# OSUrobotics/KinovaGrasping

Hardware: AMD Instinct MI355X
Metric: env-steps/sec (whole node) at 4096 envs/GPU (higher is better)
Workload: dtype f32

## Files before the change

kinovagrasping_amd/build.py:

```python
from __future__ import annotations

import os
import shutil
import subprocess
from pathlib import Path

PKG = Path(__file__).resolve().parent
CSRC = PKG / "csrc"
LIB = PKG / "libkinova_sim.so"
LIB_MG = PKG / "libkinova_sim_mg.so"
SOURCES = ["ks_api.hip", "ks_rollout.hip", "ks_mlp.hip", "ks_xchg.hip"]
HEADERS = ["ks_math.h", "ks_model.h", "ks_model_host.h", "ks_core.h", "ks_obs.h", "ks_env.h", "../../include/kinova_sim.h", "../../include/kinova_rollout.h"]


def hipcc_path() -> str:
    for cand in (os.environ.get("HIPCC"), shutil.which("hipcc"), "/opt/rocm/bin/hipcc"):
        if cand and Path(cand).exists():
            return cand
    raise RuntimeError("hipcc not found (need ROCm; this package has no CPU build)")


def needs_build(lib: Path = LIB) -> bool:
    if not lib.exists():
        return True
    t = lib.stat().st_mtime
    return any((CSRC / f).stat().st_mtime > t for f in SOURCES + HEADERS)


def build(force: bool = False, verbose: bool = False, multi_geom: bool | None = None) -> Path:
    for mg in ([False, True] if multi_geom is None else [bool(multi_geom)]):
        lib = LIB_MG if mg else LIB
        if not force and not needs_build(lib):
            continue
        cmd = [hipcc_path(), "--offload-arch=gfx950", "-O3", "-std=c++17", "-fPIC", "-shared"] + (["-DKS_MULTI_GEOM"] if mg else []) + \
              ["-o", str(lib)] + [str(CSRC / s) for s in SOURCES]
        if verbose:
            cmd.insert(1, "-Rpass-analysis=kernel-resource-usage")
        subprocess.check_call(cmd, cwd=str(CSRC))
    return LIB_MG if multi_geom else LIB
```

kinovagrasping_amd/csrc/ks_api.hip:

```cpp
#include <hip/hip_runtime.h>

#include <algorithm>
#include <cstdio>
#include <cstdlib>
#include <cstring>
#include <type_traits>
#include <map>
#include <string>
#include <vector>

#include "../../include/kinova_sim.h"
#include "ks_env.h"
#include "ks_mlp_tile.h"
#include "ks_select.h"
#include "ks_model_host.h"

using namespace ks;

namespace {

constexpr int WAVE = 64;
thread_local std::string g_create_error;

template <typename T> struct StartPool {
// ... 590 lines not shown
                wg_rays<false>(m, *bdev, N, blockIdx.x * epw, epw, (KS_LDS unsigned*)(lds + ((hull_words >> 2) << 2)) KS_RAY_PROF_ARG(nullptr));
                __threadfence_block();
                __syncthreads();
            }
            if (obs_in_step) wg_obs<false>(m, *bdev, N, blockIdx.x * epw, epw, (KS_LDS unsigned*)(lds + ((hull_words >> 2) << 2)), *out);
            if (ray_pool) {
                KS_LDS int* last = (KS_LDS int*)(lds + ((hull_words >> 2) << 2));
                __syncthreads();
                if (threadIdx.x == 0) *last = atomicAdd(&b.rayq[2], 1) == n_wg - 1;
                __syncthreads();
                if (*last) {
                    for (int i = threadIdx.x; i < 2 * n_wg; i += WG) b.rayq[4 + i] = 0;
                    if (threadIdx.x < 4) b.rayq[threadIdx.x] = 0;
                }
            }
        }
    }
}


template <typename T, bool USE_LDS>
__global__ __launch_bounds__(WG) void k_env_step(const Model<T>* __restrict__ models, Buffers<T> b, const Buffers<T>* __restrict__ bdev,
                                                   const T* __restrict__ action, int N, int frame_skip, int iters, int epw, int tap, int rays_in_step,
                                                   int pair_memory, int obs_in_step, const ObsOut<T>* __restrict__ out, int ray_pool, int n_wg) {
    env_step_body<T, USE_LDS>(models, b, bdev, action, N, frame_skip, iters, epw, tap, rays_in_step, pair_memory, obs_in_step, out, ray_pool, n_wg);
}
__global__ __launch_bounds__(WG) KS_STEP_REGS void k_env_step_f32(const Model<float>* __restrict__ models, Buffers<float> b, const Buffers<float>* __restrict__ bdev,
                                                                       const float* __restrict__ action, int N, int frame_skip, int iters, int epw, int tap, int rays_in_step,
                                                                       int pair_memory, int obs_in_step, const ObsOut<float>* __restrict__ out, int ray_pool, int n_wg) {
    env_step_body<float, true>(models, b, bdev, action, N, frame_skip, iters, epw, tap, rays_in_step, pair_memory, obs_in_step, out, ray_pool, n_wg);
}


template <int NT1, int NT2, bool EXACT = false>
__device__ __noinline__ void rollout_policy(const ks_rollout_args* __restrict__ rap, int N, int row_env, KS_LDS float* blocks) {
    const ks_rollout_args& ra = *rap;
    const int S = krsel::S, A = krsel::A;
    kmlp::f32x4(*H1)[kmlp::ROWS] = (kmlp::f32x4(*)[kmlp::ROWS])(float*)blocks;
    kmlp::f32x4(*H2)[kmlp::ROWS] = H1 + NT1 * 4;
    kmlp::f32x4(*Pp)[kmlp::ROWS] = H2 + NT2 * 4;
    const int wave = threadIdx.x >> 6, lane = threadIdx.x & 63;
    long long* vbox = (long long*)(Pp + kmlp::NW);
    for (;;) {
        if (threadIdx.x == 0) vbox[0] = (long long)__hip_atomic_load(ra.actor_ver, __ATOMIC_RELAXED, __HIP_MEMORY_SCOPE_AGENT);
        __syncthreads();
        const long long ver = vbox[0];
        __builtin_amdgcn_fence(__ATOMIC_ACQUIRE, "agent");
        const float* pw = ra.actor_pub + (ver % 3) * ra.actor_stride;
        kmlp::f32x4 z4 = {0.f, 0.f, 0.f, 0.f};
        const bool mine = kmlp::mlp3_rows16<NT1, NT2, true>(wave, lane, (long)row_env, S, 0, ra.h1, ra.h2, A, ra.obs, S, nullptr, 0, pw + ra.off_w1,
                                                            pw + ra.off_b1, pw + ra.off_w2, pw + ra.off_b2, pw + ra.off_w3, nullptr, nullptr, H1, H2, Pp,
                                                            z4);
        float y[4] = {0.f, 0.f, 0.f, 0.f};
        if (mine) {
            const float z[4] = {z4.x, z4.y, z4.z, z4.w};
            const float* b3 = pw + ra.off_b3;
#pragma unroll
            for (int i = 0; i < 4; i++) y[i] = ra.max_action / (1.f + __expf(-(z[i] + b3[i])));
        }
        __syncthreads();
        __builtin_amdgcn_fence(__ATOMIC_ACQUIRE, "agent");
        if (threadIdx.x == 0) vbox[1] = (long long)__hip_atomic_load(ra.actor_ver, __ATOMIC_RELAXED, __HIP_MEMORY_SCOPE_AGENT) - ver;
        __syncthreads();
        const bool stale = vbox[1] >= 2;
        if (stale && threadIdx.x == 0 && ra.repeats) atomicAdd((unsigned long long*)ra.repeats, 1ull);
        if (!stale) {
            if (mine) {
                float nz[4];
                krsel::normal4(ra.seed, (unsigned long long)ra.steps_total[row_env], (uint32_t)row_env, nz);
                krsel::select_one(row_env, N, y, nz, ra.obs, ra.prev_obs, ra.has_prev, ra.t, ra.ready, ra.sigma, ra.max_action, ra.skip_steps, ra.action,
                                  ra.action_t, ra.lifting);
            }
            return;
        }
        __syncthreads();
    }
}

__device__ __noinline__ void rollout_controller(const RolloutController* __restrict__ ctl, const ks_rollout_args* __restrict__ rap, int N, int row_env) {
    if (row_env < 0) return;
    const ks_rollout_args& ra = *rap;
    krsel::controller_one(row_env, N, ctl->mode, ctl->lift_rule, ra.obs, ra.prev_obs, ra.has_prev, ra.t, ra.ready, ctl->init, ra.skip_steps, ra.action,
                          ra.action_t, ra.lifting);
}
__global__ void k_controller_set(RolloutController* rec, RolloutController v, int N) {
// ... 132 lines not shown
            for (int j = 0; j < WARM_WORDS; j++) gw[q].w[j] = pair_memory ? pm[q * WARM_WORDS + j] : 0u;
        }
        lane_env_step(m, hu, *(LaneState<T>*)stp, hq, act, scr, team, snap, frame_skip, iters, ncon, status, (float*)nullptr, stp + NQ + 2 * NV, gw,
                      []() {});
        if (pair_memory) {
            KS_UNROLL
            for (int q = 0; q < WPL; q++) {
                KS_UNROLL
                for (int j = 0; j < WARM_WORDS; j++) pm[q * WARM_WORDS + j] = gw[q].w[j];
            }
        }
        team.sync();
        store_state_team<T, SUBS>(b, env, N, stp, team.sub);
        if (status) atomicOr(&b.status[env], status);
        if (team.sub == 0) b.ncon[env] = ncon;
    }
    __threadfence_block();
    __syncthreads();
    KS_RS(1)
    wg_rays<false>(m, b, N, grp * epw, epw, w KS_RAY_PROF_ARG((long long*)&rap->counters[8 + 4 * 512]));
    __threadfence_block();
    __syncthreads();
    KS_RS(2)
    wg_obs<false>(m, b, N, grp * epw, epw, w, *out);
    __threadfence_block();
    __syncthreads();
    if (active) rollout_store<float>(rap, N, env, team.sub);
    __threadfence_block();
    __syncthreads();
    KS_RS(3)
#undef KS_RS
}

__device__ __forceinline__ long long uniform64(long long v) {
    const unsigned lo = (unsigned)__builtin_amdgcn_readfirstlane((int)(unsigned)v), hi = (unsigned)__builtin_amdgcn_readfirstlane((int)(unsigned)((unsigned long long)v >> 32));
    return (long long)(((unsigned long long)hi << 32) | lo);
}
template <int NT1, int NT2>
__device__ __noinline__ void rollout_policy_wave(const ks_rollout_args* __restrict__ rap, int N, int row_env, KS_LDS float* wblocks) {
    const ks_rollout_args& ra = *rap;
    const int S = krsel::S, A = krsel::A;
    constexpr int NR = 4;
    kmlp::f32x4(*H1)[NR] = (kmlp::f32x4(*)[NR])(float*)wblocks;
    kmlp::f32x4(*H2)[NR] = H1 + NT1 * 4;
    const int lane = threadIdx.x & 63;
    for (;;) {
        const long long ver = uniform64(__hip_atomic_load(ra.actor_ver, __ATOMIC_RELAXED, __HIP_MEMORY_SCOPE_AGENT));
        __builtin_amdgcn_fence(__ATOMIC_ACQUIRE, "agent");
        const float* pw = ra.actor_pub + (ver % 3) * ra.actor_stride;
        kmlp::f32x4 z4 = {0.f, 0.f, 0.f, 0.f};
        const bool mine = kmlp::mlp3_rows_wave<NT1, NT2, true, NR>(lane, (long)row_env, S, ra.h1, ra.h2, A, ra.obs, S, pw + ra.off_w1, pw + ra.off_b1,
                                                                     pw + ra.off_w2, pw + ra.off_b2, pw + ra.off_w3, H1, H2, z4);
        float y[4] = {0.f, 0.f, 0.f, 0.f};
        if (mine) {
            const float z[4] = {z4.x, z4.y, z4.z, z4.w};
            const float* b3 = pw + ra.off_b3;
#pragma unroll
            for (int i = 0; i < 4; i++) y[i] = ra.max_action / (1.f + __expf(-(z[i] + b3[i])));
        }
        __builtin_amdgcn_fence(__ATOMIC_ACQUIRE, "agent");
        const long long ver2 = uniform64(__hip_atomic_load(ra.actor_ver, __ATOMIC_RELAXED, __HIP_MEMORY_SCOPE_AGENT));
        if (ver2 - ver < 2) {
            if (mine) {
                float nz[4];
                krsel::normal4(ra.seed, (unsigned long long)ra.steps_total[row_env], (uint32_t)row_env, nz);
                krsel::select_one(row_env, N, y, nz, ra.obs, ra.prev_obs, ra.has_prev, ra.t, ra.ready, ra.sigma, ra.max_action, ra.skip_steps, ra.action,
                                  ra.action_t, ra.lifting);
            }
            return;
        }
        if (lane == 0 && ra.repeats) atomicAdd((unsigned long long*)ra.repeats, 1ull);
    }
}

template <int NT1, int NT2>
__device__ __forceinline__ void rollout_iter_wave(const Model<float>& m, const Hulls<float>& hu, const Buffers<float>* __restrict__ bdev, int N, int frame_skip,
                                               int iters, int epw, int pair_memory, const ObsOut<float>* __restrict__ out,
                                               const ks_rollout_args* __restrict__ rap, KS_LDS float* blocks, int grp) {
    using T = float;
    using C = Crew<true>;
    const Buffers<T>& b = *bdev;
    const int wave = threadIdx.x >> 6, lane = threadIdx.x & 63;
    const int e = threadIdx.x / LANE_STRIDE;
    const Team<SUBS> team{(int)threadIdx.x % LANE_STRIDE};
    const int env = e < epw ? b.slot_env[grp * epw + e] : -1;
// ... 1106 lines not shown
            out_sent = out;
            ObsOut<T>* slot = pinned_record(capturing, h_out, (unsigned)h_out_next++, captured_out);
            if (!slot) { error = "ks_step: more captured calls than the context keeps output records for"; return KS_ERR_STATE; }
            *slot = out;
            HIPCHK(hipMemcpyAsync(d_out, slot, sizeof out, hipMemcpyHostToDevice, s));
        }
        if (timed) HIPCHK(hipEventRecord(ev0[ev_used], s));
        if constexpr (sizeof(T) == 4)
            hipLaunchKernelGGL(k_env_step_f32, dim3(n_wg), dim3(WG), step_lds, s, d_model, b, (const Buffers<T>*)d_b, (const T*)action, N,
                               cfg.frame_skip, cfg.solver_iterations, lpw, cfg.contact_tap, (int)rays_in_step, (int)(USE_LDS && cfg.pair_memory),
                               (int)obs_in_step, (const ObsOut<T>*)d_out, ray_pool, n_wg);
        else
            hipLaunchKernelGGL((k_env_step<T, USE_LDS>), dim3(n_wg), dim3(WG), step_lds, s, d_model, b, (const Buffers<T>*)d_b, (const T*)action, N,
                               cfg.frame_skip, cfg.solver_iterations, lpw, cfg.contact_tap, (int)rays_in_step, (int)(USE_LDS && cfg.pair_memory),
                               (int)obs_in_step, (const ObsOut<T>*)d_out, ray_pool, n_wg);
        if (timed) { HIPCHK(hipEventRecord(ev1[ev_used], s)); ev_used++; }
        if (!rays_in_step) hipLaunchKernelGGL((k_rays<T>), dim3((N + RAY_ENVS - 1) / RAY_ENVS, NRAY), dim3(WAVE), 0, s, d_model, b, N, 0);
        if (!obs_in_step) hipLaunchKernelGGL((k_obs<T>), dim3(blocks()), dim3(WAVE), 0, s, d_model, b, N, 0, out);
        HIPCHK(hipGetLastError());
        return KS_OK;
    }
    int check_rollout_buffers(int n_iter, const ks_rollout_args* ra) {
        if (!ra || n_iter <= 0 || (ctl_mode == 0 && (!ra->actor_pub || !ra->actor_ver)) || !ra->obs || !ra->prev_obs || !ra->has_prev || !ra->ready || !ra->lifting ||
            !ra->t || !ra->steps_total || !ra->action || !ra->action_t || !ra->reward_out || !ra->done_out || !ra->sim_obs || !ra->sim_reward ||
            !ra->sim_done || !ra->sim_info || !ra->sim_final_obs || !ra->counters) { error = "ks_rollout: NULL argument"; return KS_ERR_INVALID; }
        if (ra->with_replay && (!ra->cur_state || !ra->cur_next || !ra->cur_action || !ra->cur_reward || !ra->cur_not_done || !ra->cur_len ||
                                !ra->cur_sel || !ra->pub_len || ra->horizon <= ra->n_steps)) { error = "ks_rollout: replay buffers"; return KS_ERR_INVALID; }
        return KS_OK;
    }
    int check_rollout_actor(const ks_rollout_args* ra) {
        if (ctl_mode != 0) return KS_OK;
        if ((ra->off_w2 | ra->off_w3 | ra->actor_stride) & 3) { error = "ks_rollout: weight offsets must be multiples of 4 floats"; return KS_ERR_INVALID; }
        if ((ra->h1 | ra->h2) & 3) { error = "ks_rollout: hidden widths must be multiples of 4"; return KS_ERR_INVALID; }
        return KS_OK;
    }
    int send_rollout_records(const ks_rollout_args* ra, hipStream_t s) {
        const ObsOut<T> out{(T*)ra->sim_obs, (T*)ra->sim_reward, ra->sim_done, (T*)ra->sim_info, (T*)ra->sim_final_obs, cfg.horizon, cfg.auto_reset, cfg.obs_env_major};
        const bool capturing = stream_is_capturing(s);
        ObsOut<T>* slot = pinned_record(capturing, h_out, (unsigned)h_out_next++, captured_out);
        if (!slot) { error = "ks_rollout: more captured calls than the context keeps output records for"; return KS_ERR_STATE; }
        *slot = out;
        out_valid = false;
        HIPCHK(hipMemcpyAsync(d_out, slot, sizeof out, hipMemcpyHostToDevice, s));
        ks_rollout_args* rslot = pinned_record(capturing, h_ra, h_ra_next++, captured_ra);
        if (!rslot) { error = "ks_rollout: more captured calls than the context keeps argument records for"; return KS_ERR_STATE; }
        *rslot = *ra;
        HIPCHK(hipMemcpyAsync(d_ra, rslot, sizeof *ra, hipMemcpyHostToDevice, s));
        return KS_OK;
    }
    int rollout_exact(int n_iter, const ks_rollout_args* ra, hipStream_t s) {
#ifdef KS_MULTI_GEOM
        (void)n_iter; (void)ra; (void)s;
        error = "ks_rollout: libkinova_sim_mg.so runs fp32 contexts only (the exact mode, precision 64, is in libkinova_sim.so)";
        return KS_ERR_INVALID;
#else
        int r;
        if ((r = check_rollout_buffers(n_iter, ra))) return r;
        if (!cfg.obs_env_major || !cfg.auto_reset) { error = "ks_rollout needs env-major observations and auto_reset"; return KS_ERR_STATE; }
        if ((r = check_rollout_actor(ra))) return r;
        if (ra->budget_ticks != 0) { error = "ks_rollout: a time budget needs the wave form of the rollout kernel (ks_rollout_plan: KS_PLAN_WAVES); fp64 contexts have none"; return KS_ERR_STATE; }
        const size_t ws_offset = (step_lds + 15) / 16 * 16;
        const size_t policy_bytes = (size_t)(((ra->h1 + 15) / 16 + (ra->h2 + 15) / 16) * 4 + 4) * 16 * 16 + 16;
        const size_t lds = ws_offset + std::max(policy_bytes, (size_t)F64_RAY_BYTES);
        if (lds > 160 * 1024) { error = "ks_rollout: no LDS for the policy beside this object's hull tables"; return KS_ERR_STATE; }
        if ((r = send_rollout_records(ra, s))) return r;
        const int N = cfg.n_envs;
// ... 441 lines not shown
```

kinovagrasping_amd/csrc/ks_mlp.hip:

```cpp
#include <hip/hip_runtime.h>
#include <stdint.h>

#include <type_traits>

#include "../../include/kinova_rollout.h"
#include "../../include/kinova_sim.h"
#include "ks_mlp_tile.h"
#include "ks_select.h"

namespace {

using namespace kmlp;

#ifndef KS_SPLIT_WAVES_PER_EU
#define KS_SPLIT_WAVES_PER_EU 3
#endif

struct SelectArgs {
    const float* obs; const float* prev_obs; const uint8_t* has_prev; const int64_t* t; uint8_t* ready;
    const float* noise; unsigned long long seed; int64_t* rng_state;
    float sigma, max_action; int skip_steps;
    float* action; float* action_t; uint8_t* lifting;
};

template <int NT1, int NT2, bool VEC, bool SEL>
__global__ __launch_bounds__(64 * NW) void k_mlp3(int n, int in_a, int in_b, int h1, int h2, int out_dim, const float* __restrict__ xa, int lda,
                                              const float* __restrict__ xb, int ldb, const float* __restrict__ W1, const float* __restrict__ b1,
                                              const float* __restrict__ W2, const float* __restrict__ b2, const float* __restrict__ W3,
                                              const float* __restrict__ b3, int act, float scale, float* __restrict__ out, float* __restrict__ h1_out,
                                              float* __restrict__ h2_out, SelectArgs sel) {
    __shared__ f32x4 H1[NT1 * 4][ROWS];
    __shared__ f32x4 H2[NT2 * 4][ROWS];
    __shared__ f32x4 P[NW][ROWS];
    const int wave = threadIdx.x >> 6, lane = threadIdx.x & 63, nn = lane & 15;
    const int row = blockIdx.x * ROWS + nn;
    const bool row_ok = row < n;
    unsigned long long rng_step = 0;
    if (SEL && sel.rng_state) rng_step = (unsigned long long)sel.rng_state[0];
    f32x4 z4 = {0.f, 0.f, 0.f, 0.f};
    if (mlp3_rows16<NT1, NT2, VEC>(wave, lane, row_ok ? (long)row : -1L, in_a, in_b, h1, h2, out_dim, xa, lda, xb, ldb, W1, b1, W2, b2, W3, h1_out, h2_out,
                                   H1, H2, P, z4)) {
        const float z[4] = {z4.x, z4.y, z4.z, z4.w};
        float y[4] = {0.f, 0.f, 0.f, 0.f};
        for (int i = 0; i < out_dim; i++) {
            y[i] = z[i] + b3[i];
            if (act == KR_ACT_SIGMOID) y[i] = scale / (1.f + __expf(-y[i]));
            if (out) out[(long)row * out_dim + i] = y[i];
        }
        if (SEL) {
            float nz[4];
            if (sel.noise) {
#pragma unroll
                for (int k = 0; k < 4; k++) nz[k] = sel.noise[(long)row * 4 + k];
            } else {
                krsel::normal4(sel.seed, rng_step, (uint32_t)row, nz);
            }
            krsel::select_one(row, n, y, nz, sel.obs, sel.prev_obs, sel.has_prev, sel.t, sel.ready, sel.sigma, sel.max_action, sel.skip_steps,
                              sel.action, sel.action_t, sel.lifting);
        }
    }
    if (SEL && sel.rng_state) {
        __syncthreads();
        if (threadIdx.x == 0) {
            __threadfence();
            const unsigned ticket = atomicAdd((unsigned*)(sel.rng_state + 1), 1u);
            if (ticket == gridDim.x - 1) {
                sel.rng_state[1] = 0;
                sel.rng_state[0] = (int64_t)(rng_step + 1);
            }
        }
    }
}

template <int NT1, int NT2, bool VEC>
// ... 903 lines not shown
```

kinovagrasping_amd/csrc/ks_mlp_tile.h:

```cpp
#pragma once
#include <hip/hip_runtime.h>
#include <stdint.h>

namespace kmlp {

typedef float f32x4 __attribute__((ext_vector_type(4)));

constexpr int ROWS = 16;
constexpr int KS_IN_MAX = 6;
#ifndef KS_MLP_WAVES
#define KS_MLP_WAVES 4
#endif
constexpr int NW = KS_MLP_WAVES;

template <bool VEC> __device__ __forceinline__ f32x4 load_w4(const float* __restrict__ W, int row, int nrow, int k, int K) {
    f32x4 v = {0.f, 0.f, 0.f, 0.f};
    if (row >= nrow) return v;
    const float* p = W + (long)row * K + k;
    if (VEC && k + 3 < K) return *(const f32x4*)p;
    if (k < K) v.x = p[0];
    if (k + 1 < K) v.y = p[1];
    if (k + 2 < K) v.z = p[2];
    if (k + 3 < K) v.w = p[3];
    return v;
}

__device__ __forceinline__ f32x4 mfma4(f32x4 a, f32x4 b, f32x4 c) {
    c = __builtin_amdgcn_mfma_f32_16x16x4f32(a.x, b.x, c, 0, 0, 0);
    c = __builtin_amdgcn_mfma_f32_16x16x4f32(a.y, b.y, c, 0, 0, 0);
    c = __builtin_amdgcn_mfma_f32_16x16x4f32(a.z, b.z, c, 0, 0, 0);
    c = __builtin_amdgcn_mfma_f32_16x16x4f32(a.w, b.w, c, 0, 0, 0);
    return c;
}

__device__ __forceinline__ f32x4 bias_relu(f32x4 acc, const float* __restrict__ bias, int f, int nfeat) {
    f32x4 r;
    r.x = f < nfeat ? fmaxf(acc.x + bias[f], 0.f) : 0.f;
    r.y = f + 1 < nfeat ? fmaxf(acc.y + bias[f + 1], 0.f) : 0.f;
    r.z = f + 2 < nfeat ? fmaxf(acc.z + bias[f + 2], 0.f) : 0.f;
    r.w = f + 3 < nfeat ? fmaxf(acc.w + bias[f + 3], 0.f) : 0.f;
    return r;
}

template <int NT1, int NT2, bool VEC>
__device__ __forceinline__ bool mlp3_rows16(const int wave, const int lane, const long row, int in_a, int in_b, int h1, int h2, int out_dim,
                                            const float* __restrict__ xa, int lda, const float* __restrict__ xb, int ldb,
                                            const float* __restrict__ W1, const float* __restrict__ b1, const float* __restrict__ W2,
                                            const float* __restrict__ b2, const float* __restrict__ W3, float* __restrict__ h1_out,
                                            float* __restrict__ h2_out, f32x4 (*H1)[ROWS], f32x4 (*H2)[ROWS], f32x4 (*P)[ROWS], f32x4& z4) {
    const int nn = lane & 15, q = lane >> 4;
    const bool row_ok = row >= 0;
    const int in_dim = in_a + in_b;
    f32x4 bx[KS_IN_MAX];
#pragma unroll
    for (int s = 0; s < KS_IN_MAX; s++) {
        float v[4];
#pragma unroll
        for (int j = 0; j < 4; j++) {
            const int k = 16 * s + 4 * q + j;
            float x = 0.f;
            if (row_ok && k < in_a) x = xa[(long)row * lda + k];
            else if (row_ok && k < in_dim) x = xb[(long)row * ldb + (k - in_a)];
            v[j] = x;
        }
        bx[s] = f32x4{v[0], v[1], v[2], v[3]};
    }
    f32x4 w2[NT1];
#pragma unroll
    for (int s = 0; s < NT1; s++) w2[s] = load_w4<VEC>(W2, wave * 16 + nn, wave < NT2 ? h2 : 0, 16 * s + 4 * q, h1);
    {
        f32x4 w1[KS_IN_MAX];
#pragma unroll
        for (int s = 0; s < KS_IN_MAX; s++) w1[s] = load_w4<false>(W1, wave * 16 + nn, wave < NT1 ? h1 : 0, 16 * s + 4 * q, in_dim);
        for (int t = wave; t < NT1; t += NW) {
            f32x4 wn[KS_IN_MAX];
#pragma unroll
            for (int s = 0; s < KS_IN_MAX; s++) wn[s] = load_w4<false>(W1, (t + NW) * 16 + nn, t + NW < NT1 ? h1 : 0, 16 * s + 4 * q, in_dim);
            f32x4 acc0 = {0.f, 0.f, 0.f, 0.f}, acc1 = {0.f, 0.f, 0.f, 0.f};
#pragma unroll
            for (int s = 0; s < KS_IN_MAX; s++) {
                if (s & 1) acc1 = mfma4(w1[s], bx[s], acc1);
                else acc0 = mfma4(w1[s], bx[s], acc0);
            }
            const f32x4 hq = bias_relu(acc0 + acc1, b1, t * 16 + 4 * q, h1);
            H1[t * 4 + q][nn] = hq;
            if (h1_out && row_ok && t * 16 + 4 * q < h1) *(f32x4*)(h1_out + (long)row * h1 + t * 16 + 4 * q) = hq;
#pragma unroll
            for (int s = 0; s < KS_IN_MAX; s++) w1[s] = wn[s];
        }
    }
    __syncthreads();

    f32x4 w3[(NT2 + NW - 1) / NW];
#pragma unroll
    for (int j = 0; j < (NT2 + NW - 1) / NW; j++) w3[j] = load_w4<VEC>(W3, nn, out_dim, 16 * (wave + NW * j) + 4 * q, h2);
    for (int t = wave; t < NT2; t += NW) {
        f32x4 wn[NT1];
#pragma unroll
        for (int s = 0; s < NT1; s++) wn[s] = load_w4<VEC>(W2, (t + NW) * 16 + nn, t + NW < NT2 ? h2 : 0, 16 * s + 4 * q, h1);
        f32x4 acc0 = {0.f, 0.f, 0.f, 0.f}, acc1 = {0.f, 0.f, 0.f, 0.f};
#pragma unroll
        for (int s = 0; s < NT1; s++) {
            if (s & 1) acc1 = mfma4(w2[s], H1[s * 4 + q][nn], acc1);
            else acc0 = mfma4(w2[s], H1[s * 4 + q][nn], acc0);
        }
        const f32x4 hq = bias_relu(acc0 + acc1, b2, t * 16 + 4 * q, h2);
        H2[t * 4 + q][nn] = hq;
        if (h2_out && row_ok && t * 16 + 4 * q < h2) *(f32x4*)(h2_out + (long)row * h2 + t * 16 + 4 * q) = hq;
#pragma unroll
        for (int s = 0; s < NT1; s++) w2[s] = wn[s];
    }
    __syncthreads();

    {
        f32x4 acc = {0.f, 0.f, 0.f, 0.f};
#pragma unroll
        for (int j = 0; j < (NT2 + NW - 1) / NW; j++)
            if (wave + NW * j < NT2) acc = mfma4(w3[j], H2[(wave + NW * j) * 4 + q][nn], acc);
        if (q == 0) P[wave][nn] = acc;
    }
    __syncthreads();
    if (wave == 0 && q == 0 && row_ok) {
        z4 = P[0][nn];
#pragma unroll
        for (int w = 1; w < NW; w++) z4 += P[w][nn];
        return true;
    }
    return false;
}

template <int NT1, int NT2, bool VEC, int NR>
__device__ __forceinline__ bool mlp3_rows_wave(const int lane, const long row, int in_dim, int h1, int h2, int out_dim, const float* __restrict__ xa, int lda,
                                               const float* __restrict__ W1, const float* __restrict__ b1, const float* __restrict__ W2,
                                               const float* __restrict__ b2, const float* __restrict__ W3, f32x4 (*H1)[NR], f32x4 (*H2)[NR], f32x4& z4) {
    const int nn = lane & 15, q = lane >> 4;
    const bool row_ok = row >= 0, col_ok = nn < NR;
    const f32x4 zero = {0.f, 0.f, 0.f, 0.f};
    f32x4 bx[KS_IN_MAX];
#pragma unroll
    for (int s = 0; s < KS_IN_MAX; s++) {
        float v[4];
#pragma unroll
        for (int j = 0; j < 4; j++) {
            const int k = 16 * s + 4 * q + j;
            v[j] = (row_ok && k < in_dim) ? xa[(long)row * lda + k] : 0.f;
        }
        bx[s] = f32x4{v[0], v[1], v[2], v[3]};
    }
    f32x4 w2[NT1];
#pragma unroll
    for (int s = 0; s < NT1; s++) w2[s] = load_w4<VEC>(W2, nn, h2, 16 * s + 4 * q, h1);
    {
        f32x4 w1[KS_IN_MAX];
#pragma unroll
        for (int s = 0; s < KS_IN_MAX; s++) w1[s] = load_w4<false>(W1, nn, h1, 16 * s + 4 * q, in_dim);
        for (int t = 0; t < NT1; t++) {
            f32x4 wn[KS_IN_MAX];
#pragma unroll
            for (int s = 0; s < KS_IN_MAX; s++) wn[s] = load_w4<false>(W1, (t + 1) * 16 + nn, t + 1 < NT1 ? h1 : 0, 16 * s + 4 * q, in_dim);
            f32x4 acc0 = zero, acc1 = zero;
#pragma unroll
            for (int s = 0; s < KS_IN_MAX; s++) {
                if (s & 1) acc1 = mfma4(w1[s], bx[s], acc1);
                else acc0 = mfma4(w1[s], bx[s], acc0);
            }
            const f32x4 hq = bias_relu(acc0 + acc1, b1, t * 16 + 4 * q, h1);
            if (col_ok) H1[t * 4 + q][nn] = hq;
#pragma unroll
            for (int s = 0; s < KS_IN_MAX; s++) w1[s] = wn[s];
        }
    }
    __builtin_amdgcn_fence(__ATOMIC_RELEASE, "wavefront");
    __builtin_amdgcn_wave_barrier();
    __builtin_amdgcn_fence(__ATOMIC_ACQUIRE, "wavefront");

    f32x4 hb[NT1];
#pragma unroll
    for (int s = 0; s < NT1; s++) hb[s] = col_ok ? H1[s * 4 + q][nn] : zero;
    for (int t = 0; t < NT2; t++) {
        f32x4 wn[NT1];
#pragma unroll
        for (int s = 0; s < NT1; s++) wn[s] = load_w4<VEC>(W2, (t + 1) * 16 + nn, t + 1 < NT2 ? h2 : 0, 16 * s + 4 * q, h1);
        f32x4 acc0 = zero, acc1 = zero;
#pragma unroll
        for (int s = 0; s < NT1; s++) {
            if (s & 1) acc1 = mfma4(w2[s], hb[s], acc1);
            else acc0 = mfma4(w2[s], hb[s], acc0);
        }
        const f32x4 hq = bias_relu(acc0 + acc1, b2, t * 16 + 4 * q, h2);
        if (col_ok) H2[t * 4 + q][nn] = hq;
#pragma unroll
        for (int s = 0; s < NT1; s++) w2[s] = wn[s];
    }
    __builtin_amdgcn_fence(__ATOMIC_RELEASE, "wavefront");
    __builtin_amdgcn_wave_barrier();
    __builtin_amdgcn_fence(__ATOMIC_ACQUIRE, "wavefront");

    f32x4 part[NW];
#pragma unroll
    for (int w = 0; w < NW; w++) {
        f32x4 acc = zero;
#pragma unroll
        for (int j = 0; j < (NT2 + NW - 1) / NW; j++)
            if (w + NW * j < NT2) acc = mfma4(load_w4<VEC>(W3, nn, out_dim, 16 * (w + NW * j) + 4 * q, h2), col_ok ? H2[(w + NW * j) * 4 + q][nn] : zero, acc);
        part[w] = acc;
    }
    if (q == 0 && row_ok && col_ok) {
        z4 = part[0];
#pragma unroll
        for (int w = 1; w < NW; w++) z4 += part[w];
        return true;
    }
    return false;
}

}
```

Baseline: 2.731 million.

## Use buffer-resource loads with OOR offsets and double-buffered weight tiles in MLP

Replaces the branchy per-element global weight and input loads in the actor MLP tiles with AMD buffer-resource loads. Out-of-range lanes get an out-of-range offset so the hardware returns zero without branching. Weight and bias tiles are double-buffered (issue next tile, compute current), W3 is preloaded, and scalar parameters are forced uniform via readfirstlane. This adds a host check that observation rows fit in 32-bit byte offsets, and costs more VGPRs for the two tiles held in registers.

```diff
diff --git a/kinovagrasping_amd/build.py b/kinovagrasping_amd/build.py
--- a/kinovagrasping_amd/build.py
+++ b/kinovagrasping_amd/build.py
@@ -10,7 +10,7 @@
 LIB = PKG / "libkinova_sim.so"
 LIB_MG = PKG / "libkinova_sim_mg.so"
 SOURCES = ["ks_api.hip", "ks_rollout.hip", "ks_mlp.hip", "ks_xchg.hip"]
-HEADERS = ["ks_math.h", "ks_model.h", "ks_model_host.h", "ks_core.h", "ks_obs.h", "ks_env.h", "../../include/kinova_sim.h", "../../include/kinova_rollout.h"]
+HEADERS = ["ks_math.h", "ks_model.h", "ks_model_host.h", "ks_core.h", "ks_obs.h", "ks_env.h", "ks_mlp_tile.h", "../../include/kinova_sim.h", "../../include/kinova_rollout.h"]
 
 
 def hipcc_path() -> str:
diff --git a/kinovagrasping_amd/csrc/ks_api.hip b/kinovagrasping_amd/csrc/ks_api.hip
--- a/kinovagrasping_amd/csrc/ks_api.hip
+++ b/kinovagrasping_amd/csrc/ks_api.hip
@@ -646,6 +646,10 @@
 }
 
 
+__device__ __forceinline__ long long uniform64(long long v) {
+    const unsigned lo = (unsigned)__builtin_amdgcn_readfirstlane((int)(unsigned)v), hi = (unsigned)__builtin_amdgcn_readfirstlane((int)(unsigned)((unsigned long long)v >> 32));
+    return (long long)(((unsigned long long)hi << 32) | lo);
+}
 template <int NT1, int NT2, bool EXACT = false>
 __device__ __noinline__ void rollout_policy(const ks_rollout_args* __restrict__ rap, int N, int row_env, KS_LDS float* blocks) {
     const ks_rollout_args& ra = *rap;
@@ -658,13 +662,13 @@
     for (;;) {
         if (threadIdx.x == 0) vbox[0] = (long long)__hip_atomic_load(ra.actor_ver, __ATOMIC_RELAXED, __HIP_MEMORY_SCOPE_AGENT);
         __syncthreads();
-        const long long ver = vbox[0];
+        const long long ver = uniform64(vbox[0]);
         __builtin_amdgcn_fence(__ATOMIC_ACQUIRE, "agent");
         const float* pw = ra.actor_pub + (ver % 3) * ra.actor_stride;
         kmlp::f32x4 z4 = {0.f, 0.f, 0.f, 0.f};
-        const bool mine = kmlp::mlp3_rows16<NT1, NT2, true>(wave, lane, (long)row_env, S, 0, ra.h1, ra.h2, A, ra.obs, S, nullptr, 0, pw + ra.off_w1,
-                                                            pw + ra.off_b1, pw + ra.off_w2, pw + ra.off_b2, pw + ra.off_w3, nullptr, nullptr, H1, H2, Pp,
-                                                            z4);
+        const bool mine = kmlp::mlp3_rows16<NT1, NT2, true>(wave, lane, (long)row_env, S, 0, ra.h1, ra.h2, A, ra.obs, S, kmlp::x_bytes(N, 0, S, S), nullptr, 0,
+                                                            0u, pw + ra.off_w1, pw + ra.off_b1, pw + ra.off_w2, pw + ra.off_b2, pw + ra.off_w3, nullptr,
+                                                            nullptr, H1, H2, Pp, z4);
         float y[4] = {0.f, 0.f, 0.f, 0.f};
         if (mine) {
             const float z[4] = {z4.x, z4.y, z4.z, z4.w};
@@ -863,10 +867,6 @@
 #undef KS_RS
 }
 
-__device__ __forceinline__ long long uniform64(long long v) {
-    const unsigned lo = (unsigned)__builtin_amdgcn_readfirstlane((int)(unsigned)v), hi = (unsigned)__builtin_amdgcn_readfirstlane((int)(unsigned)((unsigned long long)v >> 32));
-    return (long long)(((unsigned long long)hi << 32) | lo);
-}
 template <int NT1, int NT2>
 __device__ __noinline__ void rollout_policy_wave(const ks_rollout_args* __restrict__ rap, int N, int row_env, KS_LDS float* wblocks) {
     const ks_rollout_args& ra = *rap;
@@ -880,8 +880,8 @@
         __builtin_amdgcn_fence(__ATOMIC_ACQUIRE, "agent");
         const float* pw = ra.actor_pub + (ver % 3) * ra.actor_stride;
         kmlp::f32x4 z4 = {0.f, 0.f, 0.f, 0.f};
-        const bool mine = kmlp::mlp3_rows_wave<NT1, NT2, true, NR>(lane, (long)row_env, S, ra.h1, ra.h2, A, ra.obs, S, pw + ra.off_w1, pw + ra.off_b1,
-                                                                     pw + ra.off_w2, pw + ra.off_b2, pw + ra.off_w3, H1, H2, z4);
+        const bool mine = kmlp::mlp3_rows_wave<NT1, NT2, true, NR>(lane, (long)row_env, S, ra.h1, ra.h2, A, ra.obs, S, kmlp::x_bytes(N, 0, S, S), pw + ra.off_w1,
+                                                                     pw + ra.off_b1, pw + ra.off_w2, pw + ra.off_b2, pw + ra.off_w3, H1, H2, z4);
         float y[4] = {0.f, 0.f, 0.f, 0.f};
         if (mine) {
             const float z[4] = {z4.x, z4.y, z4.z, z4.w};
@@ -2054,6 +2054,7 @@
         if (ctl_mode != 0) return KS_OK;
         if ((ra->off_w2 | ra->off_w3 | ra->actor_stride) & 3) { error = "ks_rollout: weight offsets must be multiples of 4 floats"; return KS_ERR_INVALID; }
         if ((ra->h1 | ra->h2) & 3) { error = "ks_rollout: hidden widths must be multiples of 4"; return KS_ERR_INVALID; }
+        if ((int64_t)cfg.n_envs * krsel::S * 4 >= (int64_t)kmlp::OOR) { error = "ks_rollout: the observation rows exceed the actor's 32-bit lane offsets"; return KS_ERR_INVALID; }
         return KS_OK;
     }
     int send_rollout_records(const ks_rollout_args* ra, hipStream_t s) {
diff --git a/kinovagrasping_amd/csrc/ks_mlp.hip b/kinovagrasping_amd/csrc/ks_mlp.hip
--- a/kinovagrasping_amd/csrc/ks_mlp.hip
+++ b/kinovagrasping_amd/csrc/ks_mlp.hip
@@ -38,8 +38,11 @@
     unsigned long long rng_step = 0;
     if (SEL && sel.rng_state) rng_step = (unsigned long long)sel.rng_state[0];
     f32x4 z4 = {0.f, 0.f, 0.f, 0.f};
-    if (mlp3_rows16<NT1, NT2, VEC>(wave, lane, row_ok ? (long)row : -1L, in_a, in_b, h1, h2, out_dim, xa, lda, xb, ldb, W1, b1, W2, b2, W3, h1_out, h2_out,
-                                   H1, H2, P, z4)) {
+    const long r0 = (long)blockIdx.x * ROWS;
+    const long nr = n - r0 < ROWS ? n - r0 : ROWS;
+    if (mlp3_rows16<NT1, NT2, VEC>(wave, lane, row_ok ? (long)nn : -1L, in_a, in_b, h1, h2, out_dim, xa + r0 * lda, lda, x_bytes(nr, 0, in_a, lda),
+                                   xb ? xb + r0 * ldb : nullptr, ldb, x_bytes(nr, in_a, in_a + in_b, ldb), W1, b1, W2, b2, W3,
+                                   h1_out ? h1_out + r0 * h1 : nullptr, h2_out ? h2_out + r0 * h2 : nullptr, H1, H2, P, z4)) {
         const float z[4] = {z4.x, z4.y, z4.z, z4.w};
         float y[4] = {0.f, 0.f, 0.f, 0.f};
         for (int i = 0; i < out_dim; i++) {
diff --git a/kinovagrasping_amd/csrc/ks_mlp_tile.h b/kinovagrasping_amd/csrc/ks_mlp_tile.h
--- a/kinovagrasping_amd/csrc/ks_mlp_tile.h
+++ b/kinovagrasping_amd/csrc/ks_mlp_tile.h
@@ -1,29 +1,86 @@
 #pragma once
+#include <stdint.h>
+
+#if defined(__HIPCC__)
 #include <hip/hip_runtime.h>
-#include <stdint.h>
+#define KS_MLP_HD __host__ __device__
+#else
+#define KS_MLP_HD
+#endif
 
 namespace kmlp {
-
-typedef float f32x4 __attribute__((ext_vector_type(4)));
 
 constexpr int ROWS = 16;
 constexpr int KS_IN_MAX = 6;
+
+constexpr uint32_t OOR = 0x7ffffff0u;
+
+KS_MLP_HD inline uint32_t tile_soff(int row0, int k0, int K) { return (uint32_t)(row0 * K + k0) * 4u; }
+KS_MLP_HD inline uint32_t quad_off(int nn, int q, int row0, int nrow, int k0, int K) {
+    const int row = row0 + nn, k = k0 + 4 * q;
+    return (row >= 0 && row < nrow && k + 3 < K) ? (uint32_t)(nn * K + 4 * q) * 4u : OOR;
+}
+KS_MLP_HD inline int tail_k(int K) { return K & ~3; }
+KS_MLP_HD inline uint32_t tail_off(int nn, int row0, int nrow, int K, int j) {
+    const int row = row0 + nn;
+    return (row >= 0 && row < nrow && j < (K & 3)) ? (uint32_t)(nn * K + tail_k(K) + j) * 4u : OOR;
+}
+KS_MLP_HD inline bool tail_here(int q, int k0, int K) { return k0 + 4 * q == tail_k(K); }
+KS_MLP_HD inline uint32_t x_off(long row, int k, int lo, int hi, int ld) {
+    return (row >= 0 && k >= lo && k < hi) ? (uint32_t)(row * ld + (k - lo)) * 4u : OOR;
+}
+KS_MLP_HD inline uint32_t x_bytes(long rows, int lo, int hi, int ld) { return rows > 0 ? (uint32_t)((rows - 1) * ld + (hi - lo)) * 4u : 0u; }
+
+}
+
+#if defined(__HIPCC__)
+namespace kmlp {
+
+typedef float f32x4 __attribute__((ext_vector_type(4)));
+typedef __amdgpu_buffer_rsrc_t rsrc_t;
+
 #ifndef KS_MLP_WAVES
 #define KS_MLP_WAVES 4
 #endif
 constexpr int NW = KS_MLP_WAVES;
 
-template <bool VEC> __device__ __forceinline__ f32x4 load_w4(const float* __restrict__ W, int row, int nrow, int k, int K) {
-    f32x4 v = {0.f, 0.f, 0.f, 0.f};
-    if (row >= nrow) return v;
-    const float* p = W + (long)row * K + k;
-    if (VEC && k + 3 < K) return *(const f32x4*)p;
-    if (k < K) v.x = p[0];
-    if (k + 1 < K) v.y = p[1];
-    if (k + 2 < K) v.z = p[2];
-    if (k + 3 < K) v.w = p[3];
-    return v;
-}
+__device__ __forceinline__ int uni(int v) { return __builtin_amdgcn_readfirstlane(v); }
+__device__ __forceinline__ const float* uni(const float* p) {
+    const unsigned long long v = (unsigned long long)p;
+    const unsigned lo = (unsigned)__builtin_amdgcn_readfirstlane((int)(unsigned)v), hi = (unsigned)__builtin_amdgcn_readfirstlane((int)(unsigned)(v >> 32));
+    return (const float*)(((unsigned long long)hi << 32) | lo);
+}
+__device__ __forceinline__ rsrc_t rsrc(const float* p, uint32_t bytes) {
+    return __builtin_amdgcn_make_buffer_rsrc(const_cast<float*>(uni(p)), 0, uni((int)bytes), 0x00020000);
+}
+__device__ __forceinline__ float ldf(rsrc_t r, uint32_t voff, uint32_t soff) { return __builtin_bit_cast(float, __builtin_amdgcn_raw_buffer_load_b32(r, (int)voff, (int)soff, 0)); }
+__device__ __forceinline__ f32x4 ldq(rsrc_t r, uint32_t voff, uint32_t soff) { return __builtin_bit_cast(f32x4, __builtin_amdgcn_raw_buffer_load_b128(r, (int)voff, (int)soff, 0)); }
+
+template <int NS, bool TAIL> struct Tile {
+    f32x4 w[NS], bq;
+    float wt[3], bt[3];
+    __device__ __forceinline__ void issue(rsrc_t rW, rsrc_t rB, int nn, int q, int row0, int nrow, int K) {
+#pragma unroll
+        for (int s = 0; s < NS; s++) w[s] = ldq(rW, quad_off(nn, q, row0, nrow, 16 * s, K), tile_soff(row0, 16 * s, K));
+        bq = ldq(rB, quad_off(0, q, 0, 1, row0, nrow), tile_soff(0, row0, nrow));
+        if (TAIL) {
+#pragma unroll
+            for (int j = 0; j < 3; j++) {
+                wt[j] = ldf(rW, tail_off(nn, row0, nrow, K, j), tile_soff(row0, 0, K));
+                bt[j] = ldf(rB, tail_off(0, 0, 1, nrow, j), 0);
+            }
+        }
+        __builtin_amdgcn_sched_barrier(0);
+    }
+    __device__ __forceinline__ f32x4 quad(int s, int q, int K) const {
+        if (TAIL && tail_here(q, 16 * s, K)) return f32x4{wt[0], wt[1], wt[2], 0.f};
+        return w[s];
+    }
+    __device__ __forceinline__ f32x4 bias(int q, int row0, int nrow) const {
+        if (TAIL && tail_here(q, row0, nrow)) return f32x4{bt[0], bt[1], bt[2], 0.f};
+        return bq;
+    }
+};
 
 __device__ __forceinline__ f32x4 mfma4(f32x4 a, f32x4 b, f32x4 c) {
     c = __builtin_amdgcn_mfma_f32_16x16x4f32(a.x, b.x, c, 0, 0, 0);
@@ -42,81 +99,114 @@
     return r;
 }
 
+__device__ __forceinline__ f32x4 bias_relu(f32x4 acc, f32x4 b, int f, int nfeat) {
+    f32x4 r;
+    r.x = f < nfeat ? fmaxf(acc.x + b.x, 0.f) : 0.f;
+    r.y = f + 1 < nfeat ? fmaxf(acc.y + b.y, 0.f) : 0.f;
+    r.z = f + 2 < nfeat ? fmaxf(acc.z + b.z, 0.f) : 0.f;
+    r.w = f + 3 < nfeat ? fmaxf(acc.w + b.w, 0.f) : 0.f;
+    return r;
+}
+
 template <int NT1, int NT2, bool VEC>
-__device__ __forceinline__ bool mlp3_rows16(const int wave, const int lane, const long row, int in_a, int in_b, int h1, int h2, int out_dim,
-                                            const float* __restrict__ xa, int lda, const float* __restrict__ xb, int ldb,
-                                            const float* __restrict__ W1, const float* __restrict__ b1, const float* __restrict__ W2,
-                                            const float* __restrict__ b2, const float* __restrict__ W3, float* __restrict__ h1_out,
-                                            float* __restrict__ h2_out, f32x4 (*H1)[ROWS], f32x4 (*H2)[ROWS], f32x4 (*P)[ROWS], f32x4& z4) {
+__device__ __forceinline__ bool mlp3_rows16(const int wave_id, const int lane, const long row, int in_a, int in_b, int h1, int h2, int out_dim,
+                                            const float* __restrict__ xa, int lda, uint32_t xa_bytes, const float* __restrict__ xb, int ldb,
+                                            uint32_t xb_bytes, const float* __restrict__ W1, const float* __restrict__ b1,
+                                            const float* __restrict__ W2, const float* __restrict__ b2, const float* __restrict__ W3,
+                                            float* __restrict__ h1_out, float* __restrict__ h2_out, f32x4 (*H1)[ROWS], f32x4 (*H2)[ROWS],
+                                            f32x4 (*P)[ROWS], f32x4& z4) {
     const int nn = lane & 15, q = lane >> 4;
+    const int wave = uni(wave_id);
     const bool row_ok = row >= 0;
+    in_a = uni(in_a), in_b = uni(in_b), h1 = uni(h1), h2 = uni(h2), out_dim = uni(out_dim), lda = uni(lda), ldb = uni(ldb);
     const int in_dim = in_a + in_b;
+    const rsrc_t rW1 = rsrc(W1, (uint32_t)(h1 * in_dim) * 4u), rB1 = rsrc(b1, (uint32_t)h1 * 4u), rW2 = rsrc(W2, (uint32_t)(h2 * h1) * 4u),
+                 rB2 = rsrc(b2, (uint32_t)h2 * 4u), rW3 = rsrc(W3, (uint32_t)(out_dim * h2) * 4u);
     f32x4 bx[KS_IN_MAX];
-#pragma unroll
-    for (int s = 0; s < KS_IN_MAX; s++) {
-        float v[4];
-#pragma unroll
-        for (int j = 0; j < 4; j++) {
-            const int k = 16 * s + 4 * q + j;
-            float x = 0.f;
-            if (row_ok && k < in_a) x = xa[(long)row * lda + k];
-            else if (row_ok && k < in_dim) x = xb[(long)row * ldb + (k - in_a)];
-            v[j] = x;
-        }
-        bx[s] = f32x4{v[0], v[1], v[2], v[3]};
-    }
-    f32x4 w2[NT1];
-#pragma unroll
-    for (int s = 0; s < NT1; s++) w2[s] = load_w4<VEC>(W2, wave * 16 + nn, wave < NT2 ? h2 : 0, 16 * s + 4 * q, h1);
-    {
-        f32x4 w1[KS_IN_MAX];
-#pragma unroll
-        for (int s = 0; s < KS_IN_MAX; s++) w1[s] = load_w4<false>(W1, wave * 16 + nn, wave < NT1 ? h1 : 0, 16 * s + 4 * q, in_dim);
-        for (int t = wave; t < NT1; t += NW) {
-            f32x4 wn[KS_IN_MAX];
-#pragma unroll
-            for (int s = 0; s < KS_IN_MAX; s++) wn[s] = load_w4<false>(W1, (t + NW) * 16 + nn, t + NW < NT1 ? h1 : 0, 16 * s + 4 * q, in_dim);
+    {
+        const rsrc_t rXa = rsrc(xa, xa_bytes);
+        float fa[KS_IN_MAX][4];
+#pragma unroll
+        for (int s = 0; s < KS_IN_MAX; s++)
+#pragma unroll
+            for (int j = 0; j < 4; j++) fa[s][j] = ldf(rXa, x_off(row, 16 * s + 4 * q + j, 0, in_a, lda), 0);
+        if (xb) {
+            const rsrc_t rXb = rsrc(xb, xb_bytes);
+#pragma unroll
+            for (int s = 0; s < KS_IN_MAX; s++)
+#pragma unroll
+                for (int j = 0; j < 4; j++) {
+                    const float fb = ldf(rXb, x_off(row, 16 * s + 4 * q + j, in_a, in_dim, ldb), 0);
+                    fa[s][j] = 16 * s + 4 * q + j < in_a ? fa[s][j] : fb;
+                }
+        }
+#pragma unroll
+        for (int s = 0; s < KS_IN_MAX; s++) bx[s] = f32x4{fa[s][0], fa[s][1], fa[s][2], fa[s][3]};
+    }
+    Tile<NT1, !VEC> a2, b2t;
+    {
+        Tile<KS_IN_MAX, true> a1, b1t;
+        a1.issue(rW1, rB1, nn, q, 16 * wave, h1, in_dim);
+        a2.issue(rW2, rB2, nn, q, 16 * wave, h2, h1);
+        auto tile1 = [&](const Tile<KS_IN_MAX, true>& w, int t) {
             f32x4 acc0 = {0.f, 0.f, 0.f, 0.f}, acc1 = {0.f, 0.f, 0.f, 0.f};
 #pragma unroll
             for (int s = 0; s < KS_IN_MAX; s++) {
-                if (s & 1) acc1 = mfma4(w1[s], bx[s], acc1);
-                else acc0 = mfma4(w1[s], bx[s], acc0);
-            }
-            const f32x4 hq = bias_relu(acc0 + acc1, b1, t * 16 + 4 * q, h1);
+                if (s & 1) acc1 = mfma4(w.quad(s, q, in_dim), bx[s], acc1);
+                else acc0 = mfma4(w.quad(s, q, in_dim), bx[s], acc0);
+            }
+            const f32x4 hq = bias_relu(acc0 + acc1, w.bias(q, 16 * t, h1), t * 16 + 4 * q, h1);
             H1[t * 4 + q][nn] = hq;
             if (h1_out && row_ok && t * 16 + 4 * q < h1) *(f32x4*)(h1_out + (long)row * h1 + t * 16 + 4 * q) = hq;
-#pragma unroll
-            for (int s = 0; s < KS_IN_MAX; s++) w1[s] = wn[s];
+        };
+#pragma unroll 1
+        for (int t = wave; t < NT1; t += 2 * NW) {
+            if (NT1 > NW) b1t.issue(rW1, rB1, nn, q, 16 * (t + NW), h1, in_dim);
+            tile1(a1, t);
+            if (NT1 > 2 * NW) a1.issue(rW1, rB1, nn, q, 16 * (t + 2 * NW), h1, in_dim);
+            if (NT1 > NW && t + NW < NT1) tile1(b1t, t + NW);
         }
     }
     __syncthreads();
 
-    f32x4 w3[(NT2 + NW - 1) / NW];
-#pragma unroll
-    for (int j = 0; j < (NT2 + NW - 1) / NW; j++) w3[j] = load_w4<VEC>(W3, nn, out_dim, 16 * (wave + NW * j) + 4 * q, h2);
-    for (int t = wave; t < NT2; t += NW) {
-        f32x4 wn[NT1];
-#pragma unroll
-        for (int s = 0; s < NT1; s++) wn[s] = load_w4<VEC>(W2, (t + NW) * 16 + nn, t + NW < NT2 ? h2 : 0, 16 * s + 4 * q, h1);
+    constexpr int NJ = (NT2 + NW - 1) / NW;
+    f32x4 w3[NJ];
+    float w3t[3];
+#pragma unroll
+    for (int j = 0; j < NJ; j++) w3[j] = ldq(rW3, quad_off(nn, q, 0, out_dim, 16 * (wave + NW * j), h2), tile_soff(0, 16 * (wave + NW * j), h2));
+    if (!VEC) {
+#pragma unroll
+        for (int j = 0; j < 3; j++) w3t[j] = ldf(rW3, tail_off(nn, 0, out_dim, h2, j), 0);
+    }
+    __builtin_amdgcn_sched_barrier(0);
+    auto tile2 = [&](const Tile<NT1, !VEC>& w, int t) {
         f32x4 acc0 = {0.f, 0.f, 0.f, 0.f}, acc1 = {0.f, 0.f, 0.f, 0.f};
 #pragma unroll
         for (int s = 0; s < NT1; s++) {
-            if (s & 1) acc1 = mfma4(w2[s], H1[s * 4 + q][nn], acc1);
-            else acc0 = mfma4(w2[s], H1[s * 4 + q][nn], acc0);
-        }
-        const f32x4 hq = bias_relu(acc0 + acc1, b2, t * 16 + 4 * q, h2);
+            if (s & 1) acc1 = mfma4(w.quad(s, q, h1), H1[s * 4 + q][nn], acc1);
+            else acc0 = mfma4(w.quad(s, q, h1), H1[s * 4 + q][nn], acc0);
+        }
+        const f32x4 hq = bias_relu(acc0 + acc1, w.bias(q, 16 * t, h2), t * 16 + 4 * q, h2);
         H2[t * 4 + q][nn] = hq;
         if (h2_out && row_ok && t * 16 + 4 * q < h2) *(f32x4*)(h2_out + (long)row * h2 + t * 16 + 4 * q) = hq;
-#pragma unroll
-        for (int s = 0; s < NT1; s++) w2[s] = wn[s];
+    };
+#pragma unroll 1
+    for (int t = wave; t < NT2; t += 2 * NW) {
+        if (NT2 > NW) b2t.issue(rW2, rB2, nn, q, 16 * (t + NW), h2, h1);
+        tile2(a2, t);
+        if (NT2 > 2 * NW) a2.issue(rW2, rB2, nn, q, 16 * (t + 2 * NW), h2, h1);
+        if (NT2 > NW && t + NW < NT2) tile2(b2t, t + NW);
     }
     __syncthreads();
 
     {
         f32x4 acc = {0.f, 0.f, 0.f, 0.f};
 #pragma unroll
-        for (int j = 0; j < (NT2 + NW - 1) / NW; j++)
-            if (wave + NW * j < NT2) acc = mfma4(w3[j], H2[(wave + NW * j) * 4 + q][nn], acc);
+        for (int j = 0; j < NJ; j++)
+            if (wave + NW * j < NT2) {
+                const f32x4 wq = (!VEC && tail_here(q, 16 * (wave + NW * j), h2)) ? f32x4{w3t[0], w3t[1], w3t[2], 0.f} : w3[j];
+                acc = mfma4(wq, H2[(wave + NW * j) * 4 + q][nn], acc);
+            }
         if (q == 0) P[wave][nn] = acc;
     }
     __syncthreads();
@@ -131,67 +221,86 @@
 
 template <int NT1, int NT2, bool VEC, int NR>
 __device__ __forceinline__ bool mlp3_rows_wave(const int lane, const long row, int in_dim, int h1, int h2, int out_dim, const float* __restrict__ xa, int lda,
-                                               const float* __restrict__ W1, const float* __restrict__ b1, const float* __restrict__ W2,
-                                               const float* __restrict__ b2, const float* __restrict__ W3, f32x4 (*H1)[NR], f32x4 (*H2)[NR], f32x4& z4) {
+                                               uint32_t xa_bytes, const float* __restrict__ W1, const float* __restrict__ b1,
+                                               const float* __restrict__ W2, const float* __restrict__ b2, const float* __restrict__ W3,
+                                               f32x4 (*H1)[NR], f32x4 (*H2)[NR], f32x4& z4) {
     const int nn = lane & 15, q = lane >> 4;
     const bool row_ok = row >= 0, col_ok = nn < NR;
     const f32x4 zero = {0.f, 0.f, 0.f, 0.f};
+    in_dim = uni(in_dim), h1 = uni(h1), h2 = uni(h2), out_dim = uni(out_dim), lda = uni(lda);
+    const rsrc_t rW1 = rsrc(W1, (uint32_t)(h1 * in_dim) * 4u), rB1 = rsrc(b1, (uint32_t)h1 * 4u), rW2 = rsrc(W2, (uint32_t)(h2 * h1) * 4u),
+                 rB2 = rsrc(b2, (uint32_t)h2 * 4u), rW3 = rsrc(W3, (uint32_t)(out_dim * h2) * 4u);
     f32x4 bx[KS_IN_MAX];
-#pragma unroll
-    for (int s = 0; s < KS_IN_MAX; s++) {
-        float v[4];
-#pragma unroll
-        for (int j = 0; j < 4; j++) {
-            const int k = 16 * s + 4 * q + j;
-            v[j] = (row_ok && k < in_dim) ? xa[(long)row * lda + k] : 0.f;
-        }
-        bx[s] = f32x4{v[0], v[1], v[2], v[3]};
-    }
-    f32x4 w2[NT1];
-#pragma unroll
-    for (int s = 0; s < NT1; s++) w2[s] = load_w4<VEC>(W2, nn, h2, 16 * s + 4 * q, h1);
-    {
-        f32x4 w1[KS_IN_MAX];
-#pragma unroll
-        for (int s = 0; s < KS_IN_MAX; s++) w1[s] = load_w4<false>(W1, nn, h1, 16 * s + 4 * q, in_dim);
-        for (int t = 0; t < NT1; t++) {
-            f32x4 wn[KS_IN_MAX];
-#pragma unroll
-            for (int s = 0; s < KS_IN_MAX; s++) wn[s] = load_w4<false>(W1, (t + 1) * 16 + nn, t + 1 < NT1 ? h1 : 0, 16 * s + 4 * q, in_dim);
+    {
+        const rsrc_t rXa = rsrc(xa, xa_bytes);
+#pragma unroll
+        for (int s = 0; s < KS_IN_MAX; s++) {
+            float v[4];
+#pragma unroll
+            for (int j = 0; j < 4; j++) v[j] = ldf(rXa, x_off(row, 16 * s + 4 * q + j, 0, in_dim, lda), 0);
+            bx[s] = f32x4{v[0], v[1], v[2], v[3]};
+        }
+    }
+    Tile<NT1, !VEC> a2, b2t;
+    {
+        Tile<KS_IN_MAX, true> a1, b1t;
+        a1.issue(rW1, rB1, nn, q, 0, h1, in_dim);
+        a2.issue(rW2, rB2, nn, q, 0, h2, h1);
+        auto tile1 = [&](const Tile<KS_IN_MAX, true>& w, int t) {
             f32x4 acc0 = zero, acc1 = zero;
 #pragma unroll
             for (int s = 0; s < KS_IN_MAX; s++) {
-                if (s & 1) acc1 = mfma4(w1[s], bx[s], acc1);
-                else acc0 = mfma4(w1[s], bx[s], acc0);
-            }
-            const f32x4 hq = bias_relu(acc0 + acc1, b1, t * 16 + 4 * q, h1);
+                if (s & 1) acc1 = mfma4(w.quad(s, q, in_dim), bx[s], acc1);
+                else acc0 = mfma4(w.quad(s, q, in_dim), bx[s], acc0);
+            }
+            const f32x4 hq = bias_relu(acc0 + acc1, w.bias(q, 16 * t, h1), t * 16 + 4 * q, h1);
             if (col_ok) H1[t * 4 + q][nn] = hq;
-#pragma unroll
-            for (int s = 0; s < KS_IN_MAX; s++) w1[s] = wn[s];
+        };
+#pragma unroll 1
+        for (int t = 0; t < NT1; t += 2) {
+            b1t.issue(rW1, rB1, nn, q, 16 * (t + 1), h1, in_dim);
+            tile1(a1, t);
+            a1.issue(rW1, rB1, nn, q, 16 * (t + 2), h1, in_dim);
+            if (t + 1 < NT1) tile1(b1t, t + 1);
         }
     }
     __builtin_amdgcn_fence(__ATOMIC_RELEASE, "wavefront");
     __builtin_amdgcn_wave_barrier();
     __builtin_amdgcn_fence(__ATOMIC_ACQUIRE, "wavefront");
 
-    f32x4 hb[NT1];
-#pragma unroll
-    for (int s = 0; s < NT1; s++) hb[s] = col_ok ? H1[s * 4 + q][nn] : zero;
-    for (int t = 0; t < NT2; t++) {
-        f32x4 wn[NT1];
-#pragma unroll
-        for (int s = 0; s < NT1; s++) wn[s] = load_w4<VEC>(W2, (t + 1) * 16 + nn, t + 1 < NT2 ? h2 : 0, 16 * s + 4 * q, h1);
+    constexpr bool HOLD_B = NT1 <= 16;
+    f32x4 hb[HOLD_B ? NT1 : 1];
+    if (HOLD_B) {
+#pragma unroll
+        for (int s = 0; s < NT1; s++) hb[s] = col_ok ? H1[s * 4 + q][nn] : zero;
+    }
+    auto tile2 = [&](const Tile<NT1, !VEC>& w, int t) {
         f32x4 acc0 = zero, acc1 = zero;
 #pragma unroll
         for (int s = 0; s < NT1; s++) {
-            if (s & 1) acc1 = mfma4(w2[s], hb[s], acc1);
-            else acc0 = mfma4(w2[s], hb[s], acc0);
-        }
-        const f32x4 hq = bias_relu(acc0 + acc1, b2, t * 16 + 4 * q, h2);
+            const f32x4 b = HOLD_B ? hb[HOLD_B ? s : 0] : (col_ok ? H1[s * 4 + q][nn] : zero);
+            if (s & 1) acc1 = mfma4(w.quad(s, q, h1), b, acc1);
+            else acc0 = mfma4(w.quad(s, q, h1), b, acc0);
+        }
+        const f32x4 hq = bias_relu(acc0 + acc1, w.bias(q, 16 * t, h2), t * 16 + 4 * q, h2);
         if (col_ok) H2[t * 4 + q][nn] = hq;
-#pragma unroll
-        for (int s = 0; s < NT1; s++) w2[s] = wn[s];
-    }
+    };
+#pragma unroll 1
+    for (int t = 0; t < NT2; t += 2) {
+        b2t.issue(rW2, rB2, nn, q, 16 * (t + 1), h2, h1);
+        tile2(a2, t);
+        a2.issue(rW2, rB2, nn, q, 16 * (t + 2), h2, h1);
+        if (t + 1 < NT2) tile2(b2t, t + 1);
+    }
+    f32x4 w3[NT2];
+    float w3t[3];
+#pragma unroll
+    for (int s = 0; s < NT2; s++) w3[s] = ldq(rW3, quad_off(nn, q, 0, out_dim, 16 * s, h2), tile_soff(0, 16 * s, h2));
+    if (!VEC) {
+#pragma unroll
+        for (int j = 0; j < 3; j++) w3t[j] = ldf(rW3, tail_off(nn, 0, out_dim, h2, j), 0);
+    }
+    __builtin_amdgcn_sched_barrier(0);
     __builtin_amdgcn_fence(__ATOMIC_RELEASE, "wavefront");
     __builtin_amdgcn_wave_barrier();
     __builtin_amdgcn_fence(__ATOMIC_ACQUIRE, "wavefront");
@@ -202,7 +311,11 @@
         f32x4 acc = zero;
 #pragma unroll
         for (int j = 0; j < (NT2 + NW - 1) / NW; j++)
-            if (w + NW * j < NT2) acc = mfma4(load_w4<VEC>(W3, nn, out_dim, 16 * (w + NW * j) + 4 * q, h2), col_ok ? H2[(w + NW * j) * 4 + q][nn] : zero, acc);
+            if (w + NW * j < NT2) {
+                const int s = w + NW * j;
+                const f32x4 wq = (!VEC && tail_here(q, 16 * s, h2)) ? f32x4{w3t[0], w3t[1], w3t[2], 0.f} : w3[s];
+                acc = mfma4(wq, col_ok ? H2[s * 4 + q][nn] : zero, acc);
+            }
         part[w] = acc;
     }
     if (q == 0 && row_ok && col_ok) {
@@ -215,3 +328,4 @@
 }
 
 }
+#endif
```

After: 2.808 million, median of 6. +2.8%, better.
